# TrustworthyComputing/helm

Hardware: AMD Instinct MI355X
Metric: encrypted gate-bootstraps/sec on AES-128 gates-mode netlist (higher is better)
Workload: dtype u32 torus (exact NTT in f64 FMA over a 49-bit prime)

## Files before the change

helm_amd/csrc/helm_hip.hip:

```cpp
#include "../../include/helm_hip.h"
#include "../../include/helm_comm.h"
#include "ntt_fp64.h"
#include "shard_rule.h"

#include <hip/hip_runtime.h>
#include <algorithm>
#include <atomic>
#include <cmath>
#include <cstdio>
#include <cstdlib>
#include <cstring>
#include <new>
#include <string>
#include <type_traits>
#include <vector>

#ifndef HELM_HIP_TU
#define HELM_HIP_TU 0
#endif
#ifndef HELM_HIP_SPLIT_TU
#define HELM_HIP_SPLIT_TU 0
#endif
using namespace helm;
struct helm_hip_wires;
struct helm_hip_program;

static thread_local std::string g_err;
static int fail(int code, const std::string &msg)
{
    g_err = msg;
    return code;
}
#if HELM_HIP_TU == 0
int helm_hip_fail_(int code, const std::string &msg) { return fail(code, msg); }
#endif
int helm_hip_runtime_guard_(const char *where);
#define HIP_TRY(expr)                                                                               \
    do {                                                                                            \
        hipError_t e__ = (expr);                                                                    \
        if (e__ != hipSuccess)                                                                      \
            return fail(HELM_ERR_HIP, std::string(#expr) + ": " + hipGetErrorString(e__));          \
    } while (0)

#define PT_TRUE 0x20000000u
#define PT_FALSE 0xE0000000u

struct PbsJob {
    int32_t op;
    int32_t which;
    int32_t in0, in1, in2;
    int32_t tv;
};

struct KsJob {
    int32_t big0, big1;
    int32_t out;
    uint32_t add_body;
};

struct LinJob {
    int32_t op, in0, out;
};

__device__ __forceinline__ uint32_t gate_lincomb(int op, int which, uint32_t l, uint32_t r, uint32_t c, bool body)
{
    const uint32_t t = body ? PT_TRUE : 0u, f = body ? PT_FALSE : 0u;
    switch (op) {
    case HELM_GATE_AND: return l + r + f;
    case HELM_GATE_OR: return l + r + t;
    case HELM_GATE_NAND: return 0u - (l + r) + t;
    case HELM_GATE_NOR: return 0u - (l + r) + f;
    case HELM_GATE_XOR: return 2u * (l + r + t);
    case HELM_GATE_XNOR: return 2u * (0u - (l + r + t));
    case HELM_GATE_MUX: return which == 0 ? (c + l + f) : (0u - c + r + f);
    default: return 0u;
    }
}

__device__ __forceinline__ uint32_t modswitch(uint32_t x, int log2_2N)
{
    uint32_t r = (x >> (32 - log2_2N - 1)) + 1u;
    return (r >> 1) & ((1u << log2_2N) - 1u);
}

__device__ __forceinline__ int decompose_step(uint32_t &state, int logB, uint32_t half_m1, int neg_B, bool last = false)
{
    const uint32_t s = state;
    const uint32_t next = last ? (s + half_m1) >> logB : (s + half_m1 + __builtin_amdgcn_ubfe(s, 2 * logB - 1, 1)) >> logB;
    state = next;
    return __mul24((int)next, neg_B) + (int)s;
}

template <int L>
__device__ __forceinline__ void decompose(uint32_t x, int logB, int (&dig)[L])
{
    const int rep = logB * L;
    uint32_t state = (x + (1u << (31 - rep))) >> (32 - rep);
    const uint32_t half_m1 = (1u << (logB - 1)) - 1u;
    const int neg_B = -(1 << logB);
#pragma unroll
    for (int lev = L - 1; lev >= 0; lev--) dig[lev] = decompose_step(state, logB, half_m1, neg_B, lev == 0);
}

static __device__ unsigned long long g_clock_probe[4];
#ifdef HELM_WIDE_STAMPS
static __device__ unsigned long long g_wide_stamps[2 * 16 * 6];
#define STAMP_DECL unsigned long long ph[6] = {0, 0, 0, 0, 0, 0}, t0 = 0, t1;
#define STAMP_BEGIN                        \
    t0 = __builtin_amdgcn_s_memtime();     \
    __builtin_amdgcn_s_waitcnt(0xC07F);
#define STAMP(k)                           \
    t1 = __builtin_amdgcn_s_memtime();     \
    __builtin_amdgcn_s_waitcnt(0xC07F);    \
    ph[k] += t1 - t0;                      \
    t0 = t1;
#define STAMP_END(wave)                                                                          \
    if ((blockIdx.x == 0 || blockIdx.x == gridDim.x - 1) && lane == 0)                           \
        for (int q = 0; q < 6; q++) g_wide_stamps[((blockIdx.x ? 1 : 0) * 16 + (wave)) * 6 + q] = ph[q];
#else
#define STAMP_DECL
#define STAMP_BEGIN
#define STAMP(k)
#define STAMP_END(wave)
#endif

enum { TW_LANE = 1 ,
       TW_LANE_FREG = 2  };

template <typename F_, int LOGN_, int K_, int L_, int TW_, int NB_ = 4>
struct PbsCfg {
    using F = F_;
    static constexpr int LOGN = LOGN_, K = K_, L = L_, TW = TW_;
    static constexpr int NB = NB_;
    static constexpr int EARLY_COLS = 2;
#ifndef HELM_PRIO_STAGES
#define HELM_PRIO_STAGES 1
#endif
    static constexpr bool PRIO_STAGES = HELM_PRIO_STAGES != 0;
    using G = Geo<LOGN>;
    static constexpr int K1 = K + 1;
    static constexpr int SLOTS = K > 1 ? K : 1;
    static constexpr int MAX_SMALL_N = 1024;
    static constexpr int SLOT_STRIDE = G::N;
    static constexpr int ACC3 = 3 * G::N - 64;
    static constexpr int WAVE_STRIDE_X = G::XPAD + (SLOTS - 1) * SLOT_STRIDE;
    static constexpr int WAVE_STRIDE = WAVE_STRIDE_X > (ACC3 + 1) / 2 ? WAVE_STRIDE_X : (ACC3 + 1) / 2;
    static constexpr int slot_off(int s) { return s == 0 ? 0 : G::XPAD + (s - 1) * SLOT_STRIDE; }
    static constexpr int TW_ROWS = G::TWB + G::TWC;
    static constexpr size_t X_OFF = 0;
    static constexpr size_t TW_OFF = X_OFF + sizeof(double) * K1 * WAVE_STRIDE;
    static constexpr size_t MS_OFF = TW_OFF + sizeof(double) * TW_ROWS * 64;
    static constexpr size_t BOOT_BYTES = (MS_OFF + sizeof(uint16_t) * (MAX_SMALL_N + 1) + 15) / 16 * 16;
    static constexpr size_t BYTES = BOOT_BYTES * NB;
};

template <typename C>
__global__ __launch_bounds__(64 * (C::K + 1) * C::NB, 1) void k_pbs(const PbsJob *__restrict__ jobs,
                                                                  const uint32_t *__restrict__ wires,
                                                                  const uint32_t *__restrict__ raw_in,
                                                                  const uint32_t *__restrict__ tvs,
                                                                  const double *__restrict__ bsk,
                                                                  const double *__restrict__ tw_fwd,
                                                                  const double *__restrict__ tw_inv,
                                                                  uint32_t *__restrict__ out_big,
                                                                  int n, int logB, int probe, int count)
{
    constexpr int LOGN = C::LOGN, K = C::K, L = C::L, NB = C::NB;
    using F = typename C::F;
    using G = Geo<LOGN>;
    constexpr int N = G::N, E = G::E, K1 = K + 1;
    extern __shared__ __align__(16) unsigned char smem_wg[];

    const int lane = threadIdx.x & 63;
    const int wv = __builtin_amdgcn_readfirstlane((int)(threadIdx.x >> 6));
    const int p = wv / NB;
    const int tid = p * 64 + lane;
    const int jix = (int)blockIdx.x * NB + wv % NB;
    if (NB > 1 && jix >= count) return;
    unsigned char *smem = smem_wg + (size_t)(wv % NB) * C::BOOT_BYTES;
    double *X = reinterpret_cast<double *>(smem + C::X_OFF);
    uint16_t *MS = reinterpret_cast<uint16_t *>(smem + C::MS_OFF);
    const PbsJob job = jobs[jix];
    const size_t row = (size_t)n + 1;

    {
        const uint32_t *a0 = nullptr, *a1 = nullptr, *a2 = nullptr;
        if (job.op < 0) a0 = raw_in + row * (size_t)job.in0;
        else {
            if (job.in0 >= 0) a0 = wires + row * (size_t)job.in0;
            if (job.in1 >= 0) a1 = wires + row * (size_t)job.in1;
            if (job.in2 >= 0) a2 = wires + row * (size_t)job.in2;
        }
        for (int i = tid; i <= n; i += 64 * K1) {
            uint32_t v;
            if (job.op < 0) v = a0[i];
            else v = gate_lincomb(job.op, job.which, a0 ? a0[i] : 0u, a1 ? a1[i] : 0u, a2 ? a2[i] : 0u, i == n);
            MS[i] = (uint16_t)modswitch(v, LOGN + 1);
        }
    }
    using TwF0 = TwLane<LOGN, false>;
    using TwF = typename std::conditional<C::TW == TW_LANE_FREG, TwLaneFwdReg<LOGN>, TwF0>::type;
    using TwI = TwLane<LOGN, true>;
    TwF0 twf0;
    TwF twf;
    TwI twi;
    {
        double *TW = reinterpret_cast<double *>(smem + C::TW_OFF);
        for (int r = p; r < C::TW_ROWS; r += K1) TW[r * 64 + lane] = tw_fwd[tw_lane_index<LOGN>(r, lane)];
        twf0.base = TW + lane;
        twi.base = TW + (63 - lane);
        twf0.fill_uniform(tw_fwd);
        twi.fill_uniform(tw_fwd);
        if constexpr (C::TW == TW_LANE) twf = twf0;
    }
    __syncthreads();
    if constexpr (C::TW == TW_LANE_FREG) twf.load(twf0);

    double *xb = X + (size_t)p * C::WAVE_STRIDE;
    uint32_t *acc_p = reinterpret_cast<uint32_t *>(xb);
    uint32_t nacc[E];
    {
        const int bt = (int)MS[n];
        const uint32_t *tv = tvs + (size_t)job.tv * N;
#pragma unroll
        for (int e = 0; e < E; e++) {
            const int j = G::jA(lane, e);
            uint32_t v = 0;
            if (p == K) {
                const int idx = (j + bt) & (2 * N - 1);
                v = tv[idx & (N - 1)];
                if (idx >= N) v = 0u - v;
            }
            nacc[e] = 0u - v;
        }
    }
    auto acc_store = [&]() {
        uint32_t *aw = acc_p + lane;
#pragma unroll
        for (int e = 0; e < E; e++) {
            const uint32_t v = 0u - nacc[e];
            aw[64 * e] = v;
            aw[64 * e + N] = nacc[e];
            if (e < E - 1) aw[64 * e + 2 * N] = v;
        }
    };
    acc_store();
    lds_wave_sync();

    const unsigned poly_bytes = (unsigned)(N / 2) * 16u;
    const unsigned step_bytes = (unsigned)(K1 * K1 * L) * poly_bytes;
    const unsigned row_off = (unsigned)(p * K1 * L) * poly_bytes;
    KeyBuf kb;
    kb.init(bsk, (size_t)n * step_bytes, lane);

    const bool stamp = (probe & 3) && blockIdx.x == gridDim.x - 1 && tid == 0;
    if (stamp) {
        g_clock_probe[0] = __builtin_amdgcn_s_memtime();
        g_clock_probe[1] = __builtin_amdgcn_s_memrealtime();
    }
    int i = 0;
    constexpr bool PRIO = NB > 1 && C::PRIO_STAGES;
    if constexpr (PRIO) __builtin_amdgcn_s_setprio(3);
    STAMP_DECL
    while (i < n) {
        STAMP_BEGIN
        const int a = __builtin_amdgcn_readfirstlane((int)MS[i]);
        const unsigned so_i = (unsigned)i * step_bytes + row_off;

        double mine[E];
        {
            uint32_t state[E];
            {
                const int rep = logB * L;
                const uint32_t *ar = acc_p + ((lane - a) & (2 * N - 1));
#pragma unroll
                for (int e = 0; e < E; e++) state[e] = (ar[64 * e] + nacc[e] + (1u << (31 - rep))) >> (32 - rep);
            }
            double keep[E];
            const uint32_t half_m1 = (1u << (logB - 1)) - 1u;
            const int neg_B = -(1 << logB);
            int cd[K1];
#pragma unroll
            for (int d = 0; d < K1; d++) cd[d] = p + d >= K1 ? p + d - K1 : p + d;
#pragma unroll
            for (int lev = L - 1; lev >= 0; lev--) {
                double x[1][E];
#pragma unroll
                for (int e = 0; e < E; e++) x[0][e] = (double)decompose_step(state[e], logB, half_m1, neg_B, lev == 0);
                double2 bwl[K1][E / 2];
                constexpr int EARLY = C::EARLY_COLS < K1 ? C::EARLY_COLS : K1;
#pragma unroll
                for (int d = 0; d < EARLY; d++)
#pragma unroll
                    for (int e2 = 0; e2 < E / 2; e2++) bwl[d][e2] = kb.load(so_i + (unsigned)(cd[d] * L + lev) * poly_bytes, e2 * 1024);
                __builtin_amdgcn_sched_barrier(0);
                ntt_forward_digits<F, LOGN, 1>(x, xb, twf, lane);
                __builtin_amdgcn_sched_barrier(0);
#pragma unroll
                for (int d = EARLY; d < K1; d++)
#pragma unroll
                    for (int e2 = 0; e2 < E / 2; e2++) bwl[d][e2] = kb.load(so_i + (unsigned)(cd[d] * L + lev) * poly_bytes, e2 * 1024);
                __builtin_amdgcn_sched_barrier(0);
                if constexpr (PRIO)
                    if (lev == 0) __builtin_amdgcn_s_setprio(0);
#pragma unroll
                for (int d = 0; d < K1; d++)
#pragma unroll
                    for (int e2 = 0; e2 < E / 2; e2++) {
                        const double2 w = bwl[d][e2];
                        const double t0 = mulmod<F>(x[0][2 * e2], w.x), t1 = mulmod<F>(x[0][2 * e2 + 1], w.y);
                        if (d == 0) {
                            mine[2 * e2] = lev == L - 1 ? t0 : mine[2 * e2] + t0;
                            mine[2 * e2 + 1] = lev == L - 1 ? t1 : mine[2 * e2 + 1] + t1;
                        } else if (d == 1) {
                            keep[2 * e2] = lev == L - 1 ? t0 : keep[2 * e2] + t0;
                            keep[2 * e2 + 1] = lev == L - 1 ? t1 : keep[2 * e2 + 1] + t1;
                        } else {
                            double *dst = xb + C::slot_off(d - 1) + lane;
                            if (lev == L - 1) {
                                dst[(2 * e2) * 64] = t0;
                                dst[(2 * e2 + 1) * 64] = t1;
                            } else {
                                lds_add(dst + (2 * e2) * 64, t0);
                                lds_add(dst + (2 * e2 + 1) * 64, t1);
                            }
                        }
                    }
                if constexpr (PRIO) {
                    if (lev == L - 1) __builtin_amdgcn_s_setprio(2);
                    else if (lev == 1) __builtin_amdgcn_s_setprio(1);
                }
            }
            {
                double *dst = xb + C::slot_off(0) + lane;
#pragma unroll
                for (int e = 0; e < E; e++) dst[e * 64] = keep[e];
            }
        }
        STAMP(0)

        lds_block_sync();
        STAMP(1)
        {
            if constexpr (!F::LAZY) {
#pragma unroll
                for (int e = 0; e < E; e++) mine[e] = reduce<F>(mine[e]);
            }
#pragma unroll
            for (int d = 1; d < K1; d++) {
                const int q = p - d < 0 ? p - d + K1 : p - d;
                const double *src = X + (size_t)q * C::WAVE_STRIDE + C::slot_off(d - 1);
#pragma unroll
                for (int e = 0; e < E; e++) mine[e] += reduce_unless_lazy<F>(src[e * 64 + lane]);
            }
        }
#pragma unroll
        for (int e = 0; e < E; e++) mine[e] = reduce<F>(mine[e]);
        STAMP(2)
        lds_block_sync();
        STAMP(3)
        if constexpr (PRIO) __builtin_amdgcn_s_setprio(3);

        ntt_inverse<F, LOGN>(mine, xb, twi, lane);
        STAMP(4)
#pragma unroll
        for (int e = 0; e < E; e++) nacc[e] -= to_torus32(mine[e]);
        acc_store();
        lds_wave_sync();
        STAMP(5)
        i++;
    }
    STAMP_END(p)

    if (stamp) {
        g_clock_probe[2] = __builtin_amdgcn_s_memtime();
        g_clock_probe[3] = __builtin_amdgcn_s_memrealtime();
    }
    uint32_t *ob = out_big + (size_t)jix * ((size_t)K * N + 1);
    if (p < K) {
#pragma unroll
        for (int e = 0; e < E; e++) {
            const int j = G::jA(lane, e);
            if (j == 0) ob[p * N] = 0u - nacc[e];
            else ob[p * N + (N - j)] = nacc[e];
        }
    } else if (lane == 0) {
        ob[K * N] = 0u - nacc[0];
    }
}

template <typename F_, int LOGN_, int K_, int L_>
struct WideCfg {
    using F = F_;
    static constexpr int LOGN = LOGN_, K = K_, L = L_, K1 = K_ + 1, NW = (K_ + 1) * L_;
    using G = Geo<LOGN>;
    static constexpr int MAX_SMALL_N = 1024;
#ifndef HELM_WIDE_PRIO
#define HELM_WIDE_PRIO 1
#endif
    static constexpr bool PRIO = HELM_WIDE_PRIO != 0;
    static constexpr int ACC3 = (3 * G::N - 64 + 1) / 2 * 2;
    static constexpr int TW_ROWS = G::TWB + G::TWC;
    static constexpr size_t X_OFF = 0;
    static constexpr size_t COL_OFF = X_OFF + sizeof(double) * NW * G::XPAD;
    static constexpr size_t TW_OFF = COL_OFF + sizeof(double) * K1 * G::N;
    static constexpr size_t ACC_OFF = TW_OFF + sizeof(double) * TW_ROWS * 64;
    static constexpr size_t MS_OFF = ACC_OFF + sizeof(uint32_t) * K1 * ACC3;
    static constexpr size_t BYTES = (MS_OFF + sizeof(uint16_t) * (MAX_SMALL_N + 1) + 15) / 16 * 16;
};

template <typename C>
__global__ __launch_bounds__(64 * C::NW, 1) void k_pbs_wide(const PbsJob *__restrict__ jobs,
                                                            const uint32_t *__restrict__ wires,
                                                            const uint32_t *__restrict__ raw_in,
                                                            const uint32_t *__restrict__ tvs,
                                                            const double *__restrict__ bsk,
                                                            const double *__restrict__ tw_fwd,
                                                            uint32_t *__restrict__ out_big, int n, int logB, int wave_map)
{
    constexpr int LOGN = C::LOGN, K = C::K, L = C::L, K1 = C::K1, NW = C::NW;
    using F = typename C::F;
    using G = Geo<LOGN>;
    constexpr int N = G::N, E = G::E;
    extern __shared__ __align__(16) unsigned char smem[];
    double *X = reinterpret_cast<double *>(smem + C::X_OFF);
    double *COL = reinterpret_cast<double *>(smem + C::COL_OFF);
    double *TW = reinterpret_cast<double *>(smem + C::TW_OFF);
    uint32_t *ACC = reinterpret_cast<uint32_t *>(smem + C::ACC_OFF);
    uint16_t *MS = reinterpret_cast<uint16_t *>(smem + C::MS_OFF);

    const int tid = threadIdx.x, lane = tid & 63;
    const int w = __builtin_amdgcn_readfirstlane(tid >> 6);
    int r = w / L, lev = w - r * L;
    if (K1 == 3 && L == 3 && (wave_map & 1)) {
        constexpr unsigned RR = 0u | 0u << 2 | 1u << 4 | 2u << 6 | 1u << 8 | 0u << 10 | 1u << 12 | 2u << 14 | 2u << 16;
        constexpr unsigned LL = 2u | 0u << 2 | 0u << 4 | 0u << 6 | 2u << 8 | 1u << 10 | 1u << 12 | 1u << 14 | 2u << 16;
        r = (int)((RR >> (2 * w)) & 3u);
        lev = (int)((LL >> (2 * w)) & 3u);
    } else if (K1 == 2 && L == 3 && (wave_map & 1)) {
        constexpr unsigned RR = 0u | 0u << 2 | 0u << 4 | 1u << 6 | 1u << 8 | 1u << 10;
        constexpr unsigned LL = 2u | 1u << 2 | 0u << 4 | 0u << 6 | 2u << 8 | 1u << 10;
        r = (int)((RR >> (2 * w)) & 3u);
        lev = (int)((LL >> (2 * w)) & 3u);
    }
    const PbsJob job = jobs[blockIdx.x];
    const size_t row = (size_t)n + 1;
    {
        const uint32_t *a0 = nullptr, *a1 = nullptr, *a2 = nullptr;
        if (job.op < 0) a0 = raw_in + row * (size_t)job.in0;
        else {
            if (job.in0 >= 0) a0 = wires + row * (size_t)job.in0;
            if (job.in1 >= 0) a1 = wires + row * (size_t)job.in1;
            if (job.in2 >= 0) a2 = wires + row * (size_t)job.in2;
        }
        for (int i = tid; i <= n; i += 64 * NW) {
            uint32_t v;
            if (job.op < 0) v = a0[i];
            else v = gate_lincomb(job.op, job.which, a0 ? a0[i] : 0u, a1 ? a1[i] : 0u, a2 ? a2[i] : 0u, i == n);
            MS[i] = (uint16_t)modswitch(v, LOGN + 1);
        }
    }
    for (int q = w; q < C::TW_ROWS; q += NW) TW[q * 64 + lane] = tw_fwd[tw_lane_index<LOGN>(q, lane)];
    for (int j = tid; j < K1 * N; j += 64 * NW) COL[j] = 0.0;
#ifndef HELM_WIDE_TW_REG
#define HELM_WIDE_TW_REG 3
#endif
    constexpr int TWR = LOGN == 9 ? HELM_WIDE_TW_REG : 0;
    TwLane<LOGN, false> twf0;
    TwLane<LOGN, true> twi0;
    twf0.base = TW + lane;
    twi0.base = TW + (63 - lane);
    twf0.fill_uniform(tw_fwd);
    twi0.fill_uniform(tw_fwd);
    __syncthreads();
    typename std::conditional<(TWR & 1) != 0, TwLaneReg<LOGN, false>, TwLane<LOGN, false>>::type twf;
    typename std::conditional<(TWR & 2) != 0, TwLaneReg<LOGN, true>, TwLane<LOGN, true>>::type twi;
    if constexpr ((TWR & 1) != 0) twf.load(twf0);
    else twf = twf0;
    if constexpr ((TWR & 2) != 0) twi.load(twi0);
    else twi = twi0;

    uint32_t *acc_r = ACC + (size_t)r * C::ACC3;
    uint32_t accr[E];
    auto acc_store = [&]() {
        uint32_t *aw = acc_r + lane;
#pragma unroll
        for (int e = 0; e < E; e++) {
            aw[64 * e] = accr[e];
            aw[64 * e + N] = 0u - accr[e];
            if (e < E - 1) aw[64 * e + 2 * N] = accr[e];
        }
    };
    if (lev == 0) {
        const int bt = (int)MS[n];
        const uint32_t *tv = tvs + (size_t)job.tv * N;
#pragma unroll
        for (int e = 0; e < E; e++) {
            uint32_t v = 0;
            if (r == K) {
                const int idx = (G::jA(lane, e) + bt) & (2 * N - 1);
                v = tv[idx & (N - 1)];
                if (idx >= N) v = 0u - v;
            }
            accr[e] = v;
        }
        acc_store();
    }
    __syncthreads();

    double *xb = X + (size_t)w * G::XPAD;
    const unsigned poly_bytes = (unsigned)(N / 2) * 16u;
    const unsigned step_bytes = (unsigned)(K1 * K1 * L) * poly_bytes;
    const unsigned wave_off = (unsigned)(r * K1 * L + lev) * poly_bytes;
    KeyBuf kb;
    kb.init(bsk, (size_t)n * step_bytes, lane);
    const uint32_t half_m1 = (1u << (logB - 1)) - 1u;
    const int neg_B = -(1 << logB);
    const int rep = logB * L;

// ... 2948 lines not shown
```

helm_amd/csrc/ntt_fp64.h:

```cpp
#pragma once
#include <hip/hip_runtime.h>
#include <stdint.h>
#include <type_traits>

namespace helm {


struct FpG {
    static constexpr double P = 661785091833857.0;
    static constexpr uint64_t P_U64 = 661785091833857ull;
    static constexpr uint64_t GEN = 3;
    static constexpr bool LAZY = true;
    static constexpr double B1 = 5072.0, B2 = 25725184.0, B3 = 130478133248.0;
};
struct FpG2 {
    static constexpr double P = 674400179654657.0;
    static constexpr uint64_t P_U64 = 674400179654657ull;
    static constexpr uint64_t GEN = 3;
    static constexpr bool LAZY = true;
    static constexpr double B1 = 5096.0, B2 = 25969216.0, B3 = 132339124736.0;
};
struct FpH {
    static constexpr double P = 1711528530149377.0;
    static constexpr uint64_t P_U64 = 1711528530149377ull;
    static constexpr uint64_t GEN = 5;
    static constexpr bool LAZY = false;
    static constexpr double B1 = 6432.0, B2 = 41370624.0, B3 = 266095853568.0;
};
struct FpI {
    static constexpr double P = 875781160960001.0;
    static constexpr uint64_t P_U64 = 875781160960001ull;
    static constexpr uint64_t GEN = 3;
    static constexpr bool LAZY = true;
    static constexpr double B1 = 5440.0, B2 = 29593600.0, B3 = 160989184000.0;
};
struct FpJ {
    static constexpr double P = 56035644604417.0;
    static constexpr uint64_t P_U64 = 56035644604417ull;
    static constexpr uint64_t GEN = 5;
    static constexpr bool LAZY = true;
    static constexpr double B1 = 2736.0, B2 = 7485696.0, B3 = 20480864256.0;
};
struct FpJ2 {
    static constexpr double P = 68035838611457.0;
    static constexpr uint64_t P_U64 = 68035838611457ull;
    static constexpr uint64_t GEN = 3;
    static constexpr bool LAZY = true;
    static constexpr double B1 = 2872.0, B2 = 8248384.0, B3 = 23689358848.0;
};
static_assert(2736ull * 2736 * 2736 * 2736 + 1 == FpJ::P_U64 && 2872ull * 2872 * 2872 * 2872 + 1 == FpJ2::P_U64, "p = b^4 + 1");
static_assert(2736ull * 2736 == 7485696ull && 7485696ull * 2736 == 20480864256ull && 2872ull * 2872 == 8248384ull &&
                  8248384ull * 2872 == 23689358848ull, "b^2, b^3");
template <typename F> struct wide_headroom : std::false_type {};
template <> struct wide_headroom<FpJ> : std::true_type {};
template <> struct wide_headroom<FpJ2> : std::true_type {};
template <typename F> struct lean_inverse_ok : std::false_type {};
template <typename F> struct has_short_roots : std::false_type {};
template <> struct has_short_roots<FpI> : std::true_type {};
template <> struct has_short_roots<FpG> : std::true_type {};
template <> struct has_short_roots<FpG2> : std::true_type {};
template <> struct has_short_roots<FpH> : std::true_type {};
template <> struct has_short_roots<FpJ> : std::true_type {};
template <> struct has_short_roots<FpJ2> : std::true_type {};
template <> struct lean_inverse_ok<FpG> : std::true_type {};
template <> struct lean_inverse_ok<FpG2> : std::true_type {};

#ifdef HELM_CHECK_BOUNDS
static __device__ unsigned int g_helm_bound_violations[8];
#define HELM_BOUND(cond, slot)                                                           \
    do {                                                                                 \
        if (!(cond)) atomicAdd(&g_helm_bound_violations[slot], 1u);                      \
    } while (0)
#else
#define HELM_BOUND(cond, slot) ((void)0)
#endif

template <typename F>
__device__ __forceinline__ double mulmod(double a, double w)
{
    constexpr double PINV = 1.0 / F::P;
    HELM_BOUND(__builtin_fabs(a) < 0x1p53, 0);
    double h = a * w;
    double l = __builtin_fma(a, w, -h);
    double q = __builtin_rint(h * PINV);
    double r = __builtin_fma(-q, F::P, h);
    return r + l;
}

template <typename F>
__device__ __forceinline__ double reduce(double a)
{
    constexpr double PINV = 1.0 / F::P;
    HELM_BOUND(__builtin_fabs(a) < 0x1p53, 1);
    double q = __builtin_rint(a * PINV);
    return __builtin_fma(-q, F::P, a);
}
template <typename F>
__device__ __forceinline__ double reduce_unless_lazy(double a)
{
    if constexpr (F::LAZY) return a;
    else return reduce<F>(a);
}

__device__ __forceinline__ uint32_t to_torus32(double v)
{
    HELM_BOUND(__builtin_fabs(v) < 0x1p51, 4);
    return (uint32_t)__double2loint(v + 6755399441055744.0 );
}

__device__ __forceinline__ void lds_wave_sync()
{
    __builtin_amdgcn_fence(__ATOMIC_ACQ_REL, "wavefront", "local");
    __builtin_amdgcn_wave_barrier();
}

__device__ __forceinline__ void lds_block_sync()
{
    __builtin_amdgcn_fence(__ATOMIC_RELEASE, "workgroup", "local");
    __builtin_amdgcn_s_barrier();
    __builtin_amdgcn_fence(__ATOMIC_ACQUIRE, "workgroup", "local");
}

typedef unsigned int u32x4_t __attribute__((ext_vector_type(4)));
struct KeyBuf {
    __amdgpu_buffer_rsrc_t rsrc;
    int lane16;
    __device__ __forceinline__ void init(const void *base, size_t bytes, int lane)
    {
        rsrc = __builtin_amdgcn_make_buffer_rsrc(const_cast<void *>(base), 0,
                                                 (int)(bytes > 0xFFFFFFFFull ? 0xFFFFFFFFull : bytes), 0x00020000);
        lane16 = lane * 16;
    }
    __device__ __forceinline__ double2 load(unsigned soff, int imm) const
    {
        const u32x4_t v = __builtin_amdgcn_raw_buffer_load_b128(rsrc, lane16 + imm, (int)soff, 0);
        double2 d;
        __builtin_memcpy(&d, &v, 16);
        return d;
    }
};

__device__ __forceinline__ void lds_add(double *p, double v)
{
    (void)__hip_atomic_fetch_add(p, v, __ATOMIC_RELAXED, __HIP_MEMORY_SCOPE_WAVEFRONT);
}

__device__ __forceinline__ void lds_add_wg(double *p, double v)
{
    (void)__hip_atomic_fetch_add(p, v, __ATOMIC_RELAXED, __HIP_MEMORY_SCOPE_WORKGROUP);
}

constexpr int ntw_count(int E, int shift, int sb_lo, int sb_hi)
{
    int c = 0;
    for (int sb = sb_lo; sb <= sb_hi; sb++) c += E >> (sb - shift + 1);
    return c;
}

template <int LOGN>
struct Geo {
    static constexpr int N = 1 << LOGN;
    static constexpr int LOGE = LOGN - 6;
    static constexpr int E = 1 << LOGE;
    static constexpr int BA = (LOGN == 9) ? 3 : 4;
    static constexpr int BC = 3;
    static constexpr int BB = LOGN - BA - BC;
    static constexpr int XPAD = N + 64;
    static_assert(LOGN == 9 || LOGN == 10 || LOGN == 11, "supported polynomial sizes");
    static_assert(BA <= LOGE && BB <= LOGE && BC <= LOGE, "block does not fit in registers");

    static constexpr int TWA = ntw_count(E, 6, LOGN - BA, LOGN - 1);
    static constexpr int TWB = ntw_count(E, BC, BC, BC + BB - 1);
    static constexpr int TWC = ntw_count(E, 0, 0, BC - 1);
    static constexpr int NTW = TWA + TWB + TWC;

    __device__ static __forceinline__ int jA(int lane, int e) { return (e << 6) | lane; }
    __device__ static __forceinline__ int jB(int lane, int e)
    {
        return ((lane >> BC) << (BC + LOGE)) | (e << BC) | (lane & ((1 << BC) - 1));
    }
    __device__ static __forceinline__ int jC(int lane, int e) { return (lane << LOGE) | e; }
    __device__ static __forceinline__ int pad1(int j) { return j + ((j >> (LOGN - 3)) << 3); }
    __device__ static __forceinline__ int pad2(int j) { return j + (j >> LOGE); }
    __device__ static __forceinline__ int baseA(int lane) { return lane; }
    __device__ static __forceinline__ int baseB(int lane)
    {
        return ((lane >> BC) << (LOGN - 3)) + ((lane >> BC) << 3) + (lane & ((1 << BC) - 1));
    }
    __device__ static __forceinline__ int baseC(int lane) { return lane * (E + 1); }
    static constexpr int offA1(int e) { return (e << 6) + ((e >> (LOGN - 9)) << 3); }
    static constexpr int offB1(int e) { return e << BC; }
    static constexpr int offB2(int e) { return (e << BC) + (e >> (LOGE - BC)); }
    static_assert(BC == 3, "the base/offset forms assume 8-lane groups in layout B");
};

struct TwMem {
    static constexpr bool MIRROR = false;
    const double *t;
    __device__ __forceinline__ double get(int, int, int, int idx, int) const { return t[idx]; }
};
template <int LOGN>
constexpr int tw_fwd_slot(int sb, int hi)
{
    using G = Geo<LOGN>;
    int slot = 0;
    for (int s = LOGN - 1; s >= LOGN - G::BA; s--) {
        if (s == sb) return slot + hi;
        slot += G::E >> (s - 6 + 1);
    }
    for (int s = G::BC + G::BB - 1; s >= G::BC; s--) {
        if (s == sb) return slot + hi;
        slot += G::E >> (s - G::BC + 1);
    }
    for (int s = G::BC - 1; s >= 0; s--) {
        if (s == sb) return slot + hi;
        slot += G::E >> (s + 1);
    }
    return -1;
}
template <int LOGN>
__device__ inline int tw_lane_index(int s, int lane)
{
    using G = Geo<LOGN>;
    int slot = 0;
    for (int sb = G::BC + G::BB - 1; sb >= G::BC; sb--) {
        const int eb = sb - G::BC, cnt = G::E >> (eb + 1);
        if (s < slot + cnt) {
            const int jh = G::jB(lane, 0) | ((s - slot) << (eb + 1 + G::BC));
            return (G::N >> (sb + 1)) + (jh >> (sb + 1));
        }
        slot += cnt;
    }
    for (int sb = G::BC - 1; sb >= 0; sb--) {
        const int cnt = G::E >> (sb + 1);
        if (s < slot + cnt) {
            const int jh = G::jC(lane, 0) | ((s - slot) << (sb + 1));
            return (G::N >> (sb + 1)) + (jh >> (sb + 1));
        }
        slot += cnt;
    }
    return 0;
}
template <int LOGN, bool MIRROR_>
struct TwLane {
    static constexpr bool MIRROR = MIRROR_;
    using G = Geo<LOGN>;
    const double *base;
    double ua[G::TWA];
    __device__ __forceinline__ double get(int sb, int hi, int cnt, int, int) const
    {
        const int fs = tw_fwd_slot<LOGN>(sb, MIRROR ? cnt - 1 - hi : hi);
        if (fs < G::TWA) return ua[fs];
        return base[(fs - G::TWA) * 64];
    }
    __device__ __forceinline__ void fill_uniform(const double *__restrict__ table)
    {
        int slot = 0;
#pragma unroll
        for (int sb = LOGN - 1; sb >= LOGN - G::BA; sb--) {
#pragma unroll
            for (int hi = 0; hi < (G::E >> (sb - 6 + 1)); hi++) ua[slot++] = table[(G::N >> (sb + 1)) + hi];
        }
    }
};

template <int LOGN, bool MIRROR_ = false>
struct TwLaneReg {
    static constexpr bool MIRROR = MIRROR_;
    using G = Geo<LOGN>;
    double ua[G::TWA];
    double c[G::TWB + G::TWC];
    __device__ __forceinline__ void load(const TwLane<LOGN, MIRROR_> &t)
    {
#pragma unroll
        for (int r = 0; r < G::TWA; r++) ua[r] = t.ua[r];
#pragma unroll
        for (int r = 0; r < G::TWB + G::TWC; r++) c[r] = t.base[r * 64];
    }
    __device__ __forceinline__ double get(int sb, int hi, int cnt, int, int) const
    {
        const int fs = tw_fwd_slot<LOGN>(sb, MIRROR ? cnt - 1 - hi : hi);
        if (fs < G::TWA) return ua[fs];
        return c[fs - G::TWA];
    }
};
template <int LOGN> using TwLaneFwdReg = TwLaneReg<LOGN, false>;

template <int LOGN, bool MIRROR_>
struct TwHybrid {
    static constexpr bool MIRROR = MIRROR_;
    using G = Geo<LOGN>;
    const double *t;
    const double *base;
    __device__ __forceinline__ double get(int sb, int hi, int cnt, int idx, int) const
    {
        if (sb < G::BC) {
            const int fs = tw_fwd_slot<LOGN>(sb, MIRROR ? cnt - 1 - hi : hi) - G::TWA - G::TWB;
            return base[fs * 64];
        }
        return t[MIRROR ? 3 * (G::N >> (sb + 1)) - 1 - idx : idx];
    }
};

template <int LOGN, bool MIRROR_>
struct TwHybridC {
    static constexpr bool MIRROR = MIRROR_;
    using G = Geo<LOGN>;
    const double *t;
    double c[G::TWC];
    __device__ __forceinline__ void load(const double *base)
    {
#pragma unroll
        for (int r = 0; r < G::TWC; r++) c[r] = base[r * 64];
    }
    __device__ __forceinline__ double get(int sb, int hi, int cnt, int idx, int) const
    {
        if (sb < G::BC) return c[tw_fwd_slot<LOGN>(sb, MIRROR ? cnt - 1 - hi : hi) - G::TWA - G::TWB];
        return t[MIRROR ? 3 * (G::N >> (sb + 1)) - 1 - idx : idx];
    }
};

template <typename F, int LOGN, int M, int SHIFT, int SB_HI, int SB_LO, int SLOT0, typename TW, bool PLAIN_TOP = false>
__device__ __forceinline__ void fwd_block(double (&x)[M][Geo<LOGN>::E], const TW &tw, int jbase)
{
    static_assert(!PLAIN_TOP || SB_HI == LOGN - 1, "the short twiddle is the first stage's");
    constexpr int E = Geo<LOGN>::E, N = Geo<LOGN>::N;
    int slot = SLOT0;
#pragma unroll
    for (int sb = SB_HI; sb >= SB_LO; sb--) {
        const int eb = sb - SHIFT;
#pragma unroll
        for (int hi = 0; hi < (E >> (eb + 1)); hi++) {
            const int jh = jbase | (hi << (eb + 1 + SHIFT));
            const double w = tw.get(sb, hi, E >> (eb + 1), (N >> (sb + 1)) + (jh >> (sb + 1)), slot++);
#pragma unroll
            for (int lo = 0; lo < (1 << eb); lo++) {
                const int e0 = (hi << (eb + 1)) | lo, e1 = e0 | (1 << eb);
#pragma unroll
                for (int m = 0; m < M; m++) {
                    double U = x[m][e0], V = (PLAIN_TOP && sb == SB_HI) ? x[m][e1] * w : mulmod<F>(x[m][e1], w);
                    x[m][e0] = U + V;
                    x[m][e1] = U - V;
                    HELM_BOUND(__builtin_fabs(x[m][e0]) < 0x1p53 && __builtin_fabs(x[m][e1]) < 0x1p53, 2);
                }
            }
        }
    }
}

template <typename F, int LOGN, int SHIFT, int SB_LO, int SB_HI, int SLOT0, typename TW>
__device__ __forceinline__ void inv_block(double (&x)[Geo<LOGN>::E], const TW &tw, int jbase)
{
    constexpr int E = Geo<LOGN>::E, N = Geo<LOGN>::N;
    int slot = SLOT0;
#pragma unroll
    for (int sb = SB_LO; sb <= SB_HI; sb++) {
        const int eb = sb - SHIFT;
        if (!F::LAZY && sb - SB_LO == 2 && SB_HI - SB_LO == 3) {
#pragma unroll
            for (int e = 0; e < E; e++) x[e] = reduce<F>(x[e]);
        }
#pragma unroll
        for (int hi = 0; hi < (E >> (eb + 1)); hi++) {
            const int jh = jbase | (hi << (eb + 1 + SHIFT));
            const double w = tw.get(sb, hi, E >> (eb + 1), (N >> (sb + 1)) + (jh >> (sb + 1)), slot++);
#pragma unroll
            for (int lo = 0; lo < (1 << eb); lo++) {
                const int e0 = (hi << (eb + 1)) | lo, e1 = e0 | (1 << eb);
                double U = x[e0], V = x[e1];
                x[e0] = U + V;
                HELM_BOUND(__builtin_fabs(x[e0]) < 0x1p53 && __builtin_fabs(U - V) < 0x1p53, 2);
                x[e1] = mulmod<F>(TW::MIRROR ? V - U : U - V, w);
            }
        }
    }
}

struct NoHook {
    __device__ __forceinline__ void operator()() const {}
};
template <typename F, int M, int E>
__device__ __forceinline__ void fwd_top2_digits(double (&x)[M][E])
{
    constexpr int Q = E / 4;
#pragma unroll
    for (int m = 0; m < M; m++)
#pragma unroll
        for (int e = 0; e < Q; e++) {
            const double d0 = x[m][e], d2 = x[m][e + Q], d4 = x[m][e + 2 * Q], d6 = x[m][e + 3 * Q];
            const double a0 = __builtin_fma(d4, F::B2, d0), a4 = __builtin_fma(d4, -F::B2, d0);
            const double u = __builtin_fma(d6, F::B3, d2 * F::B1), v = __builtin_fma(d6, F::B1, d2 * F::B3);
            x[m][e] = a0 + u;
            x[m][e + Q] = a0 - u;
            x[m][e + 2 * Q] = a4 + v;
            x[m][e + 3 * Q] = a4 - v;
            [[maybe_unused]] constexpr double LIM = wide_headroom<F>::value ? 0x1p52 : F::P * 0.5;
            HELM_BOUND(__builtin_fabs(x[m][e]) < LIM && __builtin_fabs(x[m][e + Q]) < LIM &&
                           __builtin_fabs(x[m][e + 2 * Q]) < LIM && __builtin_fabs(x[m][e + 3 * Q]) < LIM, 2);
        }
}

template <typename F, int LOGN, int M, typename TW, int PRIO = 0, typename HOOK = NoHook, int DIGITS = 0>
__device__ __forceinline__ void ntt_forward(double (&x)[M][Geo<LOGN>::E], double *xbuf, const TW &tw, int lane,
                                            const HOOK &before_last = HOOK())
{
    using G = Geo<LOGN>;
    if constexpr (DIGITS == 1 && has_short_roots<F>::value)
        fwd_block<F, LOGN, M, 6, LOGN - 1, LOGN - G::BA, 0, TW, true>(x, tw, G::jA(lane, 0));
    else if constexpr (DIGITS == 2 && has_short_roots<F>::value) {
        static_assert(G::BA >= 3, "stages 1 and 2 pair slots e, e + E/2 and e, e + E/4 of block A");
        fwd_top2_digits<F, M, G::E>(x);
        fwd_block<F, LOGN, M, 6, LOGN - 3, LOGN - G::BA, 3>(x, tw, G::jA(lane, 0));
    } else if constexpr (DIGITS == 3 && has_short_roots<F>::value) {
        static_assert(G::BA >= 2, "the caller has done stride bit LOGN-1 of block A");
        fwd_block<F, LOGN, M, 6, LOGN - 2, LOGN - G::BA, 1>(x, tw, G::jA(lane, 0));
    } else
        fwd_block<F, LOGN, M, 6, LOGN - 1, LOGN - G::BA, 0>(x, tw, G::jA(lane, 0));
    if constexpr (PRIO > 0) __builtin_amdgcn_s_setprio(PRIO - 1);
    double *pA = xbuf + G::baseA(lane), *pB = xbuf + G::baseB(lane), *pC = xbuf + G::baseC(lane);
    constexpr bool SKIP_T1 = (DIGITS == 2 || DIGITS == 3) && has_short_roots<F>::value && G::BB == 3;
    static_assert(!SKIP_T1 || (G::BA >= 3 && G::BB == 3), "SKIP_T1: block A ends below 1.2 p only behind fwd_top2_digits, and block B must be three stages");
#pragma unroll
    for (int m = 0; m < M; m++)
#pragma unroll
        for (int e = 0; e < G::E; e++) pA[m * G::XPAD + G::offA1(e)] = SKIP_T1 ? x[m][e] : reduce_unless_lazy<F>(x[m][e]);
    lds_wave_sync();
#pragma unroll
    for (int m = 0; m < M; m++)
#pragma unroll
        for (int e = 0; e < G::E; e++) x[m][e] = pB[m * G::XPAD + G::offB1(e)];
    lds_wave_sync();
    fwd_block<F, LOGN, M, G::BC, G::BC + G::BB - 1, G::BC, G::TWA>(x, tw, G::jB(lane, 0));
    if constexpr (PRIO > 1) __builtin_amdgcn_s_setprio(PRIO - 2);
#pragma unroll
    for (int m = 0; m < M; m++)
#pragma unroll
        for (int e = 0; e < G::E; e++) pB[m * G::XPAD + G::offB2(e)] = reduce_unless_lazy<F>(x[m][e]);
    lds_wave_sync();
#pragma unroll
    for (int m = 0; m < M; m++)
#pragma unroll
        for (int e = 0; e < G::E; e++) x[m][e] = pC[m * G::XPAD + e];
    lds_wave_sync();
    before_last();
    fwd_block<F, LOGN, M, 0, G::BC - 1, 0, G::TWA + G::TWB>(x, tw, G::jC(lane, 0));
}

#ifndef HELM_SHORT_ROOT_STAGES
#define HELM_SHORT_ROOT_STAGES 1
#endif
template <typename F, int LOGN, int M, int PRIO = 0, typename TW>
__device__ __forceinline__ void ntt_forward_digits(double (&x)[M][Geo<LOGN>::E], double *xbuf, const TW &tw, int lane)
{
    ntt_forward<F, LOGN, M, TW, PRIO, NoHook, HELM_SHORT_ROOT_STAGES != 0 ? 2 : 0>(x, xbuf, tw, lane);
}

template <typename F, int LOGN, typename TW, int PRIO = 0, bool CENTRE = true, typename HOOK = NoHook>
__device__ __forceinline__ void ntt_inverse(double (&x)[Geo<LOGN>::E], double *xbuf, const TW &tw, int lane,
                                            const HOOK &before_write = HOOK())
{
    using G = Geo<LOGN>;
#ifndef HELM_LEAN_INVERSE
#define HELM_LEAN_INVERSE 1
#endif
    constexpr bool LEAN = HELM_LEAN_INVERSE != 0 && F::LAZY && lean_inverse_ok<F>::value && CENTRE && LOGN == 9 && G::BA == 3 && G::BB == 3 && G::BC == 3;
    static_assert(!LEAN || (G::E == 8 && G::BA + G::BB + G::BC == LOGN), "LEAN inverse: slot-class bounds are derived for Geo<9>");
    constexpr bool WIDE = wide_headroom<F>::value && LOGN == 9 && G::BA == 3 && G::BB == 3 && G::BC == 3;
    if constexpr (LEAN) {
#pragma unroll
        for (int e = 0; e < G::E; e++) HELM_BOUND(__builtin_fabs(x[e]) <= F::P * 0.5000001, 3);
    }
    if constexpr (WIDE) {
#pragma unroll
        for (int e = 0; e < G::E; e++) HELM_BOUND(__builtin_fabs(x[e]) <= F::P * 4.5, 3);
    }
    inv_block<F, LOGN, 0, 0, G::BC - 1, 0>(x, tw, G::jC(lane, 0));
    before_write();
    if constexpr (PRIO > 0) __builtin_amdgcn_s_setprio(PRIO - 1);
    double *pA = xbuf + G::baseA(lane), *pB = xbuf + G::baseB(lane), *pC = xbuf + G::baseC(lane);
#pragma unroll
    for (int e = 0; e < G::E; e++) pC[e] = ((LEAN && e >= 3) || (WIDE && e >= 1)) ? x[e] : reduce<F>(x[e]);
    lds_wave_sync();
#pragma unroll
    for (int e = 0; e < G::E; e++) x[e] = pB[G::offB2(e)];
    lds_wave_sync();
    inv_block<F, LOGN, G::BC, G::BC, G::BC + G::BB - 1, G::TWC>(x, tw, G::jB(lane, 0));
    if constexpr (PRIO > 1) __builtin_amdgcn_s_setprio(PRIO - 2);
#pragma unroll
    for (int e = 0; e < G::E; e++) pB[G::offB1(e)] = ((LEAN && e >= 5) || (WIDE && e >= 1)) ? x[e] : reduce<F>(x[e]);
    lds_wave_sync();
#pragma unroll
    for (int e = 0; e < G::E; e++) x[e] = pA[G::offA1(e)];
    lds_wave_sync();
    inv_block<F, LOGN, 6, LOGN - G::BA, LOGN - 1, G::TWC + G::TWB>(x, tw, G::jA(lane, 0));
    if constexpr (CENTRE) {
#pragma unroll
        for (int e = 0; e < G::E; e++) x[e] = reduce<F>(x[e]);
    } else if constexpr (WIDE) {
    } else if constexpr (G::BA == 4) {
        static_assert(F::LAZY, "uncentred outputs need the headroom of the 49-bit fields");
        x[0] = reduce<F>(x[0]);
    }
}

}
```

Measured before the change: 132,100.

## Rewrite NTT blocks B and C as twisted 8-point transforms with short-root multiplies

```diff
diff --git a/helm_amd/csrc/helm_hip.hip b/helm_amd/csrc/helm_hip.hip
--- a/helm_amd/csrc/helm_hip.hip
+++ b/helm_amd/csrc/helm_hip.hip
@@ -147,6 +147,11 @@
     static constexpr int WAVE_STRIDE = WAVE_STRIDE_X > (ACC3 + 1) / 2 ? WAVE_STRIDE_X : (ACC3 + 1) / 2;
     static constexpr int slot_off(int s) { return s == 0 ? 0 : G::XPAD + (s - 1) * SLOT_STRIDE; }
     static constexpr int TW_ROWS = G::TWB + G::TWC;
+#ifndef HELM_BLK8
+#define HELM_BLK8 1
+#endif
+    static constexpr bool BLK8 = HELM_BLK8 != 0 && blk8_field<F>::value && LOGN == 9 && TW == TW_LANE_FREG;
+    static_assert(!BLK8 || TW_ROWS == 14, "the table holds the 2 x 7 block-form twiddles of the inverse");
     static constexpr size_t X_OFF = 0;
     static constexpr size_t TW_OFF = X_OFF + sizeof(double) * K1 * WAVE_STRIDE;
     static constexpr size_t MS_OFF = TW_OFF + sizeof(double) * TW_ROWS * 64;
@@ -199,22 +204,29 @@
         }
     }
     using TwF0 = TwLane<LOGN, false>;
-    using TwF = typename std::conditional<C::TW == TW_LANE_FREG, TwLaneFwdReg<LOGN>, TwF0>::type;
-    using TwI = TwLane<LOGN, true>;
+    using TwF = typename std::conditional<C::BLK8, TwBlk8Fwd<LOGN>,
+                                          typename std::conditional<C::TW == TW_LANE_FREG, TwLaneFwdReg<LOGN>, TwF0>::type>::type;
+    using TwI = typename std::conditional<C::BLK8, TwBlk8Inv<LOGN>, TwLane<LOGN, true>>::type;
     TwF0 twf0;
     TwF twf;
     TwI twi;
     {
         double *TW = reinterpret_cast<double *>(smem + C::TW_OFF);
-        for (int r = p; r < C::TW_ROWS; r += K1) TW[r * 64 + lane] = tw_fwd[tw_lane_index<LOGN>(r, lane)];
+        for (int r = p; r < C::TW_ROWS; r += K1) {
+            if constexpr (C::BLK8) TW[r * 64 + lane] = tw_blk8_row<LOGN, -1>(tw_fwd, r, lane);
+            else TW[r * 64 + lane] = tw_fwd[tw_lane_index<LOGN>(r, lane)];
+        }
         twf0.base = TW + lane;
         twi.base = TW + (63 - lane);
         twf0.fill_uniform(tw_fwd);
         twi.fill_uniform(tw_fwd);
-        if constexpr (C::TW == TW_LANE) twf = twf0;
+        if constexpr (C::BLK8) {
+            twi.row = TW + lane;
+            twf.load(tw_fwd, lane);
+        } else if constexpr (C::TW == TW_LANE) twf = twf0;
     }
     __syncthreads();
-    if constexpr (C::TW == TW_LANE_FREG) twf.load(twf0);
+    if constexpr (!C::BLK8 && C::TW == TW_LANE_FREG) twf.load(twf0);
 
     double *xb = X + (size_t)p * C::WAVE_STRIDE;
     uint32_t *acc_p = reinterpret_cast<uint32_t *>(xb);
diff --git a/helm_amd/csrc/ntt_fp64.h b/helm_amd/csrc/ntt_fp64.h
--- a/helm_amd/csrc/ntt_fp64.h
+++ b/helm_amd/csrc/ntt_fp64.h
@@ -64,6 +64,8 @@
 template <> struct has_short_roots<FpJ2> : std::true_type {};
 template <> struct lean_inverse_ok<FpG> : std::true_type {};
 template <> struct lean_inverse_ok<FpG2> : std::true_type {};
+template <typename F> struct blk8_field : std::false_type {};
+template <> struct blk8_field<FpG> : std::true_type {};
 
 #ifdef HELM_CHECK_BOUNDS
 static __device__ unsigned int g_helm_bound_violations[8];
@@ -95,6 +97,20 @@
     double q = __builtin_rint(a * PINV);
     return __builtin_fma(-q, F::P, a);
 }
+template <typename F, int K>
+__device__ __forceinline__ double mul_broot(double x)
+{
+    static_assert(has_short_roots<F>::value && K >= 1 && K <= 7 && K != 4, "b^K, K = 1..7 except -1");
+    constexpr int J = K & 3;
+    constexpr double BJ = J == 1 ? F::B1 : J == 2 ? F::B2 : F::B3;
+    constexpr double BC = J == 1 ? F::B3 : J == 2 ? F::B2 : F::B1;
+    constexpr double BC_INV = 1.0 / BC;
+    HELM_BOUND(__builtin_fabs(x) < 0x1p53, 0);
+    const double q = __builtin_rint(x * BC_INV);
+    const double x0 = __builtin_fma(-q, BC, x);
+    return K < 4 ? __builtin_fma(x0, BJ, -q) : __builtin_fma(x0, -BJ, q);
+}
+
 template <typename F>
 __device__ __forceinline__ double reduce_unless_lazy(double a)
 {
@@ -320,6 +336,57 @@
     }
 };
 
+template <int LOGN>
+__device__ __forceinline__ double tw_pow(const double *__restrict__ tw_fwd, int x)
+{
+    constexpr int N = 1 << LOGN;
+    x &= 2 * N - 1;
+    const double v = tw_fwd[__builtin_bitreverse32((unsigned)(x & (N - 1))) >> (32 - LOGN)];
+    return (x & N) ? -v : v;
+}
+template <int LOGN, int SIGN>
+__device__ inline double tw_blk8_row(const double *__restrict__ tw_fwd, int r, int lane)
+{
+    using G = Geo<LOGN>;
+    static_assert(G::E == 8 && G::BB == 3 && G::BC == 3, "blocks B and C are 8-groups");
+    const int blk = r >= 7, t = r - 7 * blk + 1;
+    const int s = blk ? 0 : G::BC;
+    const int j = blk ? G::jC(lane, 0) : G::jB(lane, 0);
+    const int a = (int)(__builtin_bitreverse32((unsigned)((G::N >> (s + 1)) + (j >> (s + 1)))) >> (32 - LOGN));
+    return tw_pow<LOGN>(tw_fwd, SIGN * t * a);
+}
+template <int LOGN>
+struct TwBlk8Fwd {
+    static constexpr bool MIRROR = false;
+    static constexpr bool BLK8 = true;
+    using G = Geo<LOGN>;
+    double ua[G::TWA];
+    double w[14];
+    __device__ __forceinline__ void load(const double *__restrict__ tw_fwd, int lane)
+    {
+        TwLane<LOGN, false> u;
+        u.fill_uniform(tw_fwd);
+#pragma unroll
+        for (int r = 0; r < G::TWA; r++) ua[r] = u.ua[r];
+#pragma unroll
+        for (int r = 0; r < 14; r++) w[r] = tw_blk8_row<LOGN, 1>(tw_fwd, r, lane);
+    }
+    __device__ __forceinline__ double get(int sb, int hi, int, int, int) const
+    {
+        const int fs = tw_fwd_slot<LOGN>(sb, hi);
+        return ua[fs < G::TWA ? fs : 0];
+    }
+    __device__ __forceinline__ double pw(int blk, int t) const { return w[7 * blk + t - 1]; }
+};
+template <int LOGN>
+struct TwBlk8Inv : TwLane<LOGN, true> {
+    static constexpr bool BLK8 = true;
+    const double *row;
+    __device__ __forceinline__ double pw(int blk, int t) const { return row[(7 * blk + t - 1) * 64]; }
+};
+template <typename TW, typename = void> struct is_blk8 : std::false_type {};
+template <typename TW> struct is_blk8<TW, std::void_t<decltype(TW::BLK8)>> : std::bool_constant<TW::BLK8> {};
+
 template <typename F, int LOGN, int M, int SHIFT, int SB_HI, int SB_LO, int SLOT0, typename TW, bool PLAIN_TOP = false>
 __device__ __forceinline__ void fwd_block(double (&x)[M][Geo<LOGN>::E], const TW &tw, int jbase)
 {
@@ -348,9 +415,10 @@
     }
 }
 
-template <typename F, int LOGN, int SHIFT, int SB_LO, int SB_HI, int SLOT0, typename TW>
+template <typename F, int LOGN, int SHIFT, int SB_LO, int SB_HI, int SLOT0, typename TW, bool SHORT_TOP = false>
 __device__ __forceinline__ void inv_block(double (&x)[Geo<LOGN>::E], const TW &tw, int jbase)
 {
+    static_assert(!SHORT_TOP || (SHIFT == 6 && SB_HI == LOGN - 1 && SB_LO <= LOGN - 2), "block A: twiddles lane-uniform");
     constexpr int E = Geo<LOGN>::E, N = Geo<LOGN>::N;
     int slot = SLOT0;
 #pragma unroll
@@ -363,17 +431,106 @@
 #pragma unroll
         for (int hi = 0; hi < (E >> (eb + 1)); hi++) {
             const int jh = jbase | (hi << (eb + 1 + SHIFT));
-            const double w = tw.get(sb, hi, E >> (eb + 1), (N >> (sb + 1)) + (jh >> (sb + 1)), slot++);
+            const bool short_stage = SHORT_TOP && sb >= LOGN - 2;
+            const double w = short_stage ? 0.0 : tw.get(sb, hi, E >> (eb + 1), (N >> (sb + 1)) + (jh >> (sb + 1)), slot);
+            slot++;
 #pragma unroll
             for (int lo = 0; lo < (1 << eb); lo++) {
                 const int e0 = (hi << (eb + 1)) | lo, e1 = e0 | (1 << eb);
                 double U = x[e0], V = x[e1];
                 x[e0] = U + V;
                 HELM_BOUND(__builtin_fabs(x[e0]) < 0x1p53 && __builtin_fabs(U - V) < 0x1p53, 2);
+                if constexpr (SHORT_TOP) {
+                    if (short_stage) {
+                        x[e1] = sb == LOGN - 1 ? mul_broot<F, 6>(U - V) : hi == 0 ? mul_broot<F, 7>(U - V) : mul_broot<F, 5>(U - V);
+                        continue;
+                    }
+                }
                 x[e1] = mulmod<F>(TW::MIRROR ? V - U : U - V, w);
             }
         }
     }
+}
+
+template <typename F, int LOGN, int M, int BLK, bool X0C, typename TW>
+__device__ __forceinline__ void fwd_blk8(double (&x)[M][Geo<LOGN>::E], const TW &tw)
+{
+    static_assert(Geo<LOGN>::E == 8, "one 8-group per lane");
+#pragma unroll
+    for (int m = 0; m < M; m++) {
+        double z[8];
+        z[0] = X0C ? reduce<F>(x[m][0]) : x[m][0];
+#pragma unroll
+        for (int t = 1; t < 8; t++) z[t] = mulmod<F>(x[m][t], tw.pw(BLK, t));
+        double a[8], c[8];
+#pragma unroll
+        for (int e = 0; e < 4; e++) {
+            a[e] = z[e] + z[e + 4];
+            a[e + 4] = z[e] - z[e + 4];
+        }
+        const double t6 = mul_broot<F, 2>(a[6]), t7 = mul_broot<F, 2>(a[7]);
+        c[0] = a[0] + a[2];
+        c[2] = a[0] - a[2];
+        c[1] = a[1] + a[3];
+        c[3] = a[1] - a[3];
+        c[4] = a[4] + t6;
+        c[6] = a[4] - t6;
+        c[5] = a[5] + t7;
+        c[7] = a[5] - t7;
+        const double u3 = mul_broot<F, 2>(c[3]), u5 = mul_broot<F, 1>(c[5]), u7 = mul_broot<F, 3>(c[7]);
+        x[m][0] = c[0] + c[1];
+        x[m][1] = c[0] - c[1];
+        x[m][2] = c[2] + u3;
+        x[m][3] = c[2] - u3;
+        x[m][4] = c[4] + u5;
+        x[m][5] = c[4] - u5;
+        x[m][6] = c[6] + u7;
+        x[m][7] = c[6] - u7;
+#ifdef HELM_CHECK_BOUNDS
+        bool ok = true;
+        for (int e = 0; e < 8; e++)
+            ok = ok && __builtin_fabs(a[e]) < 0x1p53 && __builtin_fabs(c[e]) < 0x1p53 && __builtin_fabs(x[m][e]) < 0x1p53;
+        HELM_BOUND(ok, 2);
+#endif
+    }
+}
+
+template <typename F, int LOGN, int BLK, typename TW>
+__device__ __forceinline__ void inv_blk8(double (&x)[Geo<LOGN>::E], const TW &tw)
+{
+    static_assert(Geo<LOGN>::E == 8, "one 8-group per lane");
+    double c[8], a[8];
+    c[0] = x[0] + x[1];
+    c[1] = x[0] - x[1];
+    c[2] = x[2] + x[3];
+    c[3] = mul_broot<F, 6>(x[2] - x[3]);
+    c[4] = x[4] + x[5];
+    c[5] = mul_broot<F, 7>(x[4] - x[5]);
+    c[6] = x[6] + x[7];
+    c[7] = mul_broot<F, 5>(x[6] - x[7]);
+    a[0] = c[0] + c[2];
+    a[2] = c[0] - c[2];
+    a[1] = c[1] + c[3];
+    a[3] = c[1] - c[3];
+    a[4] = c[4] + c[6];
+    a[6] = mul_broot<F, 6>(c[4] - c[6]);
+    a[5] = c[5] + c[7];
+    a[7] = mul_broot<F, 6>(c[5] - c[7]);
+#ifdef HELM_CHECK_BOUNDS
+    bool ok = true;
+    for (int e = 0; e < 8; e++) ok = ok && __builtin_fabs(c[e]) < 0x1p53 && __builtin_fabs(a[e]) < 0x1p53;
+    HELM_BOUND(ok && __builtin_fabs(x[2] - x[3]) < 0x1p53 && __builtin_fabs(x[4] - x[5]) < 0x1p53 &&
+                   __builtin_fabs(x[6] - x[7]) < 0x1p53 && __builtin_fabs(c[4] - c[6]) < 0x1p53 && __builtin_fabs(c[5] - c[7]) < 0x1p53,
+               2);
+#endif
+#pragma unroll
+    for (int e = 0; e < 4; e++) {
+        x[e] = a[e] + a[e + 4];
+        x[e + 4] = a[e] - a[e + 4];
+        HELM_BOUND(__builtin_fabs(x[e]) < 0x1p53 && __builtin_fabs(x[e + 4]) < 0x1p53, 2);
+    }
+#pragma unroll
+    for (int t = 1; t < 8; t++) x[t] = mulmod<F>(x[t], tw.pw(BLK, t));
 }
 
 struct NoHook {
@@ -405,6 +562,9 @@
                                             const HOOK &before_last = HOOK())
 {
     using G = Geo<LOGN>;
+    constexpr bool BLK8 = is_blk8<TW>::value;
+    static_assert(!BLK8 || (blk8_field<F>::value && F::LAZY && DIGITS == 2 && LOGN == 9 && G::BA == 3 && G::BB == 3 && G::BC == 3),
+                  "8-point block form: N = 512 transforms of digits in a field of blk8_field");
     if constexpr (DIGITS == 1 && has_short_roots<F>::value)
         fwd_block<F, LOGN, M, 6, LOGN - 1, LOGN - G::BA, 0, TW, true>(x, tw, G::jA(lane, 0));
     else if constexpr (DIGITS == 2 && has_short_roots<F>::value) {
@@ -430,7 +590,8 @@
 #pragma unroll
         for (int e = 0; e < G::E; e++) x[m][e] = pB[m * G::XPAD + G::offB1(e)];
     lds_wave_sync();
-    fwd_block<F, LOGN, M, G::BC, G::BC + G::BB - 1, G::BC, G::TWA>(x, tw, G::jB(lane, 0));
+    if constexpr (BLK8) fwd_blk8<F, LOGN, M, 0, false>(x, tw);
+    else fwd_block<F, LOGN, M, G::BC, G::BC + G::BB - 1, G::BC, G::TWA>(x, tw, G::jB(lane, 0));
     if constexpr (PRIO > 1) __builtin_amdgcn_s_setprio(PRIO - 2);
 #pragma unroll
     for (int m = 0; m < M; m++)
@@ -443,7 +604,8 @@
         for (int e = 0; e < G::E; e++) x[m][e] = pC[m * G::XPAD + e];
     lds_wave_sync();
     before_last();
-    fwd_block<F, LOGN, M, 0, G::BC - 1, 0, G::TWA + G::TWB>(x, tw, G::jC(lane, 0));
+    if constexpr (BLK8) fwd_blk8<F, LOGN, M, 1, true>(x, tw);
+    else fwd_block<F, LOGN, M, 0, G::BC - 1, 0, G::TWA + G::TWB>(x, tw, G::jC(lane, 0));
 }
 
 #ifndef HELM_SHORT_ROOT_STAGES
@@ -463,10 +625,13 @@
 #ifndef HELM_LEAN_INVERSE
 #define HELM_LEAN_INVERSE 1
 #endif
-    constexpr bool LEAN = HELM_LEAN_INVERSE != 0 && F::LAZY && lean_inverse_ok<F>::value && CENTRE && LOGN == 9 && G::BA == 3 && G::BB == 3 && G::BC == 3;
+    constexpr bool BLK8 = is_blk8<TW>::value;
+    static_assert(!BLK8 || (blk8_field<F>::value && F::LAZY && CENTRE && LOGN == 9 && G::BA == 3 && G::BB == 3 && G::BC == 3),
+                  "8-point block form: N = 512, centred output, a field of blk8_field");
+    constexpr bool LEAN = !BLK8 && HELM_LEAN_INVERSE != 0 && F::LAZY && lean_inverse_ok<F>::value && CENTRE && LOGN == 9 && G::BA == 3 && G::BB == 3 && G::BC == 3;
     static_assert(!LEAN || (G::E == 8 && G::BA + G::BB + G::BC == LOGN), "LEAN inverse: slot-class bounds are derived for Geo<9>");
     constexpr bool WIDE = wide_headroom<F>::value && LOGN == 9 && G::BA == 3 && G::BB == 3 && G::BC == 3;
-    if constexpr (LEAN) {
+    if constexpr (LEAN || BLK8) {
 #pragma unroll
         for (int e = 0; e < G::E; e++) HELM_BOUND(__builtin_fabs(x[e]) <= F::P * 0.5000001, 3);
     }
@@ -474,25 +639,27 @@
 #pragma unroll
         for (int e = 0; e < G::E; e++) HELM_BOUND(__builtin_fabs(x[e]) <= F::P * 4.5, 3);
     }
-    inv_block<F, LOGN, 0, 0, G::BC - 1, 0>(x, tw, G::jC(lane, 0));
+    if constexpr (BLK8) inv_blk8<F, LOGN, 1>(x, tw);
+    else inv_block<F, LOGN, 0, 0, G::BC - 1, 0>(x, tw, G::jC(lane, 0));
     before_write();
     if constexpr (PRIO > 0) __builtin_amdgcn_s_setprio(PRIO - 1);
     double *pA = xbuf + G::baseA(lane), *pB = xbuf + G::baseB(lane), *pC = xbuf + G::baseC(lane);
 #pragma unroll
-    for (int e = 0; e < G::E; e++) pC[e] = ((LEAN && e >= 3) || (WIDE && e >= 1)) ? x[e] : reduce<F>(x[e]);
+    for (int e = 0; e < G::E; e++) pC[e] = ((LEAN && e >= 3) || ((WIDE || BLK8) && e >= 1)) ? x[e] : reduce<F>(x[e]);
     lds_wave_sync();
 #pragma unroll
     for (int e = 0; e < G::E; e++) x[e] = pB[G::offB2(e)];
     lds_wave_sync();
-    inv_block<F, LOGN, G::BC, G::BC, G::BC + G::BB - 1, G::TWC>(x, tw, G::jB(lane, 0));
+    if constexpr (BLK8) inv_blk8<F, LOGN, 0>(x, tw);
+    else inv_block<F, LOGN, G::BC, G::BC, G::BC + G::BB - 1, G::TWC>(x, tw, G::jB(lane, 0));
     if constexpr (PRIO > 1) __builtin_amdgcn_s_setprio(PRIO - 2);
 #pragma unroll
-    for (int e = 0; e < G::E; e++) pB[G::offB1(e)] = ((LEAN && e >= 5) || (WIDE && e >= 1)) ? x[e] : reduce<F>(x[e]);
+    for (int e = 0; e < G::E; e++) pB[G::offB1(e)] = ((LEAN && e >= 5) || ((WIDE || BLK8) && e >= 1)) ? x[e] : reduce<F>(x[e]);
     lds_wave_sync();
 #pragma unroll
     for (int e = 0; e < G::E; e++) x[e] = pA[G::offA1(e)];
     lds_wave_sync();
-    inv_block<F, LOGN, 6, LOGN - G::BA, LOGN - 1, G::TWC + G::TWB>(x, tw, G::jA(lane, 0));
+    inv_block<F, LOGN, 6, LOGN - G::BA, LOGN - 1, G::TWC + G::TWB, TW, BLK8>(x, tw, G::jA(lane, 0));
     if constexpr (CENTRE) {
 #pragma unroll
         for (int e = 0; e < G::E; e++) x[e] = reduce<F>(x[e]);
```

New measurement: 138,000, median of 6. 1.05x the previous value.
